# SysCV/sam-pt

Hardware: NVIDIA H100
Metric: frames/sec, SAM-PT hot path (PIPS track + SAM ViT encode + prompt/mask decode w/ 12 refinements) (higher is better)
Workload: dtype f16 hi.hi + two e4m3 correction passes (~fp32 products) qkv/MLP, f16 hi+lo x3 elsewhere ViT; f32 PIPS + decoder

## Files before the change

### sam-pt_b200/csrc/decoder.cu

```cuda
#include <cstdlib>

#include "common.cuh"
#include "kernels.cuh"
#include "tc_api.cuh"
#include "../../include/sampt_b200.h"

namespace sampt {

#define SKIP_RETURN(skip) \
  if ((skip) != nullptr && *(skip) != 0) return;

struct PromptArgs {
  const float* coords;
  const int* labels;
  int K;
  const float* box;
  int use_box;
  const float* gauss;
  const float* pt_emb[4];
  const float* not_a_point;
  const float* out_tokens;
  int n_out_tok;
  float img_size;
};
// ... 586 lines not shown
    const int w = threadIdx.x >> 5;
    if ((threadIdx.x & 31) == 0) { sred[0][w] = xmin; sred[1][w] = ymin; sred[2][w] = xmax; sred[3][w] = ymax; sred[4][w] = cnt; }
    __syncthreads();
    if (threadIdx.x == 0) {
      for (int k = 1; k < 8; ++k) {
        sred[0][0] = min(sred[0][0], sred[0][k]); sred[1][0] = min(sred[1][0], sred[1][k]);
        sred[2][0] = max(sred[2][0], sred[2][k]); sred[3][0] = max(sred[3][0], sred[3][k]);
        sred[4][0] += sred[4][k];
      }
      if (sred[4][0] > 0) {
        atomicMin(&bbox[0], sred[0][0]); atomicMin(&bbox[1], sred[1][0]);
        atomicMax(&bbox[2], sred[2][0]); atomicMax(&bbox[3], sred[3][0]);
        atomicAdd(&bbox[4], sred[4][0]);
      }
    }
  }
}
__global__ void refine_ctl_kernel(int* bbox, float* box_out, int* skip, int* n_done) {
  if (*skip == 0) {
    if (bbox[4] < 2) *skip = 1;
    else {
      box_out[0] = (float)bbox[0]; box_out[1] = (float)bbox[1]; box_out[2] = (float)bbox[2]; box_out[3] = (float)bbox[3];
      if (n_done) *n_done += 1;
    }
  }
  bbox[0] = 0x7fffffff; bbox[1] = 0x7fffffff; bbox[2] = -1; bbox[3] = -1; bbox[4] = 0;
}
__global__ void init_ctl_kernel(int* bbox, int* skip, int* n_done) {
  bbox[0] = 0x7fffffff; bbox[1] = 0x7fffffff; bbox[2] = -1; bbox[3] = -1; bbox[4] = 0;
  *skip = 0;
  if (n_done) *n_done = 0;
}

struct AttnW {
  const float *qw, *qb, *kw, *kb, *vw, *vb, *ow, *ob; int internal;
  const __half *qw16 = nullptr, *kw16 = nullptr, *vw16 = nullptr, *ow16 = nullptr;
};
struct LayerW {
  AttnW self_attn, t2i, i2t;
  const float *n1w, *n1b, *n2w, *n2b, *n3w, *n3b, *n4w, *n4b;
  const float *l1w, *l1b, *l2w, *l2b;
  const float *pek_t2i, *peq_i2t;
};
struct DecW {
  LayerW layer[2];
  AttnW final_attn; const float *nfw, *nfb, *pek_final;
  const float *up0_w , *up0_b4 ;
  const __half* up0_w16 = nullptr;
  bool tc = false;
  const float *up_lnw, *up_lnb, *up3_w, *up3_b;
  Mlp3Job hyper[4], iou;
  DenseW dense;
  PromptArgs prompt;
  int n_out_tok;
  int hq = 0;
  Mlp3Job hq_mlp;
  const float *mf0_w, *mf0_b, *mf_lnw, *mf_lnb, *mf3_w, *mf3_b;
  const float *enc0_w, *enc0_b4, *enc_lnw, *enc_lnb, *enc3_w, *enc3_b;
  const float *cv0_w, *cv0_b4, *cv_lnw, *cv_lnb, *cv3_w, *cv3_b;
  int vit_dim = 0;
};

static int load_attn(Ctx* c, const std::string& p, AttnW* a, int internal) {
  a->internal = internal;
  SAMPT_TRY(get_f32(c, p + "q_proj.weight", &a->qw)); SAMPT_TRY(get_f32(c, p + "q_proj.bias", &a->qb));
  SAMPT_TRY(get_f32(c, p + "k_proj.weight", &a->kw)); SAMPT_TRY(get_f32(c, p + "k_proj.bias", &a->kb));
  SAMPT_TRY(get_f32(c, p + "v_proj.weight", &a->vw)); SAMPT_TRY(get_f32(c, p + "v_proj.bias", &a->vb));
  SAMPT_TRY(get_f32(c, p + "out_proj.weight", &a->ow)); SAMPT_TRY(get_f32(c, p + "out_proj.bias", &a->ob));
  return 0;
}
static bool decoder_tc_enabled() {
  static const int on = [] { const char* e = std::getenv("SAMPT_DECODER_TC"); return (e != nullptr && e[0] == '0') ? 0 : 1; }();
  return on != 0;
}
static int load_w16(Ctx* c, const std::string& name, const __half** out) { return get_f16(c, name, out); }
static int load_mlp3(Ctx* c, const std::string& p, Mlp3Job* j, int n_out) {
  SAMPT_TRY(get_f32(c, p + "layers.0.weight", &j->w0)); SAMPT_TRY(get_f32(c, p + "layers.0.bias", &j->b0));
  SAMPT_TRY(get_f32(c, p + "layers.1.weight", &j->w1)); SAMPT_TRY(get_f32(c, p + "layers.1.bias", &j->b1));
  SAMPT_TRY(get_f32(c, p + "layers.2.weight", &j->w2)); SAMPT_TRY(get_f32(c, p + "layers.2.bias", &j->b2));
  j->n_out = n_out;
  return 0;
}
static int load_dec(Ctx* c, DecW* w) {
  const std::string md = "sam.mask_decoder.", tr = md + "transformer.", pe = "sam.prompt_encoder.";
  for (int i = 0; i < 2; ++i) {
    const std::string lp = tr + "layers." + std::to_string(i) + ".";
    LayerW& L = w->layer[i];
    SAMPT_TRY(load_attn(c, lp + "self_attn.", &L.self_attn, 256));
    SAMPT_TRY(load_attn(c, lp + "cross_attn_token_to_image.", &L.t2i, 128));
    SAMPT_TRY(load_attn(c, lp + "cross_attn_image_to_token.", &L.i2t, 128));
    SAMPT_TRY(get_f32(c, lp + "norm1.weight", &L.n1w)); SAMPT_TRY(get_f32(c, lp + "norm1.bias", &L.n1b));
    SAMPT_TRY(get_f32(c, lp + "norm2.weight", &L.n2w)); SAMPT_TRY(get_f32(c, lp + "norm2.bias", &L.n2b));
    SAMPT_TRY(get_f32(c, lp + "norm3.weight", &L.n3w)); SAMPT_TRY(get_f32(c, lp + "norm3.bias", &L.n3b));
    SAMPT_TRY(get_f32(c, lp + "norm4.weight", &L.n4w)); SAMPT_TRY(get_f32(c, lp + "norm4.bias", &L.n4b));
    SAMPT_TRY(get_f32(c, lp + "mlp.lin1.weight", &L.l1w)); SAMPT_TRY(get_f32(c, lp + "mlp.lin1.bias", &L.l1b));
    SAMPT_TRY(get_f32(c, lp + "mlp.lin2.weight", &L.l2w)); SAMPT_TRY(get_f32(c, lp + "mlp.lin2.bias", &L.l2b));
    SAMPT_TRY(get_f32(c, lp + "pek_t2i", &L.pek_t2i)); SAMPT_TRY(get_f32(c, lp + "peq_i2t", &L.peq_i2t));
  }
  SAMPT_TRY(load_attn(c, tr + "final_attn_token_to_image.", &w->final_attn, 128));
  w->tc = decoder_tc_enabled() && c->find(md + "output_upscaling.0.w16") != nullptr;
  if (w->tc) {
    for (int i = 0; i < 2; ++i) {
      const std::string lp = tr + "layers." + std::to_string(i) + ".";
      SAMPT_TRY(load_w16(c, lp + "cross_attn_token_to_image.k_proj.w16", &w->layer[i].t2i.kw16));
      SAMPT_TRY(load_w16(c, lp + "cross_attn_token_to_image.v_proj.w16", &w->layer[i].t2i.vw16));
      SAMPT_TRY(load_w16(c, lp + "cross_attn_image_to_token.q_proj.w16", &w->layer[i].i2t.qw16));
      SAMPT_TRY(load_w16(c, lp + "cross_attn_image_to_token.out_proj.w16", &w->layer[i].i2t.ow16));
    }
// ... 51 lines not shown
  int T;
};

#define LAUNCH_OK() do { c->launches++; SAMPT_LAUNCH_CHECK(); } while (0)

static int sg(Ctx* c, cudaStream_t st, const float* X, int ldx, const float* W, const float* b, const float* resid, int ldr,
              float* Y, int ldy, int M, int N, int K, int act, const int* skip) {
  return sgemm_nt_skip(c, st, X, ldx, W, K, b, resid, ldr, Y, ldy, M, N, K, act, skip);
}

__global__ void __launch_bounds__(256)
split_f32_kernel(const float* __restrict__ x, __half* __restrict__ out, long long n4 , int K, const int* skip) {
  SKIP_RETURN(skip);
  const long long i = (long long)blockIdx.x * 256 + threadIdx.x;
  if (i >= n4) return;
  const long long e = i * 4;
  const long long r = e / K;
  const int cidx = (int)(e % K);
  const float4 v = *reinterpret_cast<const float4*>(x + e);
  const __half2 h0 = __floats2half2_rn(v.x, v.y), h1 = __floats2half2_rn(v.z, v.w);
  const float2 f0 = __half22float2(h0), f1 = __half22float2(h1);
  const __half2 l0 = __floats2half2_rn(v.x - f0.x, v.y - f0.y), l1 = __floats2half2_rn(v.z - f1.x, v.w - f1.y);
  __half* o = out + r * 2 * K + cidx;
  *reinterpret_cast<uint2*>(o) = make_uint2(*reinterpret_cast<const uint32_t*>(&h0), *reinterpret_cast<const uint32_t*>(&h1));
  *reinterpret_cast<uint2*>(o + K) = make_uint2(*reinterpret_cast<const uint32_t*>(&l0), *reinterpret_cast<const uint32_t*>(&l1));
}
static int split_rows(Ctx* c, cudaStream_t st, const float* x, __half* out, int rows, int K, const int* skip) {
  const long long n4 = (long long)rows * K / 4;
  split_f32_kernel<<<cdiv(n4, 256), 256, 0, st>>>(x, out, n4, K, skip);
  c->launches++;
  SAMPT_LAUNCH_CHECK();
  return 0;
}
static int tcg(Ctx* c, cudaStream_t st, const __half* X16, const __half* W16, const float* b, const float* resid, float* Y, int ldy,
               int M, int N, int K, const int* skip) {
  GemmSeg seg{};
  seg.nseg = 3;
  seg.a_off[0] = 0; seg.b_off[0] = 0;
  seg.a_off[1] = K; seg.b_off[1] = 0;
  seg.a_off[2] = 0; seg.b_off[2] = K;
  GemmEpi ep{};
  ep.out32 = Y; ep.ldc = ldy; ep.bias = b; ep.resid = resid; ep.skip = skip;
  return gemm_tc(c, st, X16, 2 * K, W16, 2 * K, M, N, K, seg, ep);
}

static int launch_tok_self(Ctx* c, cudaStream_t st, int kind, const float* q, const float* k, const float* v, float* out, int T,
                           const int* skip) {
  if (kind == 1) {
    const size_t smem = ((size_t)2 * T * 33 + (size_t)8 * T + 8 * 32) * sizeof(float);
    SAMPT_CHECK(smem <= 200 * 1024, "too many prompt tokens (%d) for the token self-attention", T);
    SAMPT_TRY(ensure_func_smem(c, "attn_tok_self_kernel<32>", attn_tok_self_kernel<32>, 200 * 1024));
    attn_tok_self_kernel<32><<<dim3(cdiv(T, 32), 8), 256, smem, st>>>(q, k, v, out, T, 8, skip);
  } else {
    attn_q_small_kernel<32><<<dim3(T, 8), 256, 0, st>>>(q, k, v, out, T, 8, skip);
  }
  LAUNCH_OK();
  return 0;
}
static int launch_t2i(Ctx* c, cudaStream_t st, const float* q, const float* k, const float* v, float* part, float* out, int T, int Nk,
                      const int* skip) {
  constexpr int KPS = 256;
  const int nsplit = (Nk + KPS - 1) / KPS;
  attn_t2i_partial_kernel<16, KPS><<<dim3(nsplit, 8), 256, 0, st>>>(q, k, v, part, T, Nk, 8, skip);
  LAUNCH_OK();
  attn_t2i_combine_kernel<16><<<cdiv(T * 128, 128), 128, 0, st>>>(part, out, T, 8, nsplit, skip);
  LAUNCH_OK();
  return 0;
}
static int launch_i2t(Ctx* c, cudaStream_t st, const float* q, const float* k, const float* v, float* out, int N, int T, const int* skip) {
  attn_kv_small_kernel<16><<<cdiv((long long)cdiv(N, 32) * 8, 8), 256, 0, st>>>(q, k, v, out, N, T, 8, skip);
  LAUNCH_OK();
  return 0;
}

static int attn_tok_to_img(Ctx* c, cudaStream_t st, const AttnW& a, const float* q_in, const float* keys, const float* pek,
                           DecBufs& b, float* out , const float* resid, int GG, const int* skip) {
  const int T = b.T;
  SAMPT_TRY(sg(c, st, q_in, 256, a.qw, a.qb, nullptr, 0, b.tq, 128, T, 128, 256, 0, skip));
  if (a.kw16 != nullptr) {
    SAMPT_TRY(tcg(c, st, b.keys16, a.kw16, a.kb, pek, b.ik, 128, GG, 128, 256, skip));
    SAMPT_TRY(tcg(c, st, b.keys16, a.vw16, a.vb, nullptr, b.iv, 128, GG, 128, 256, skip));
  } else {
    SAMPT_TRY(sg(c, st, keys, 256, a.kw, a.kb, pek, 128, b.ik, 128, GG, 128, 256, 0, skip));
    SAMPT_TRY(sg(c, st, keys, 256, a.vw, a.vb, nullptr, 0, b.iv, 128, GG, 128, 256, 0, skip));
  }
  SAMPT_TRY(launch_t2i(c, st, b.tq, b.ik, b.iv, b.part, b.ta, T, GG, skip));
  SAMPT_TRY(sg(c, st, b.ta, 128, a.ow, a.ob, resid, 256, out, 256, T, 256, 128, 0, skip));
  return 0;
}

static int two_way_layer(Ctx* c, cudaStream_t st, const LayerW& L, int idx, DecBufs& b, int GG, const int* skip) {
  const int T = b.T;
  if (idx == 0) {
    SAMPT_TRY(sg(c, st, b.queries, 256, L.self_attn.qw, L.self_attn.qb, nullptr, 0, b.tq, 256, T, 256, 256, 0, skip));
    SAMPT_TRY(sg(c, st, b.queries, 256, L.self_attn.kw, L.self_attn.kb, nullptr, 0, b.tk, 256, T, 256, 256, 0, skip));
  } else {
    add_kernel<<<cdiv(T * 64, 256), 256, 0, st>>>(b.queries, b.tokens, b.qpe, (long long)T * 64, skip);
    LAUNCH_OK();
    SAMPT_TRY(sg(c, st, b.qpe, 256, L.self_attn.qw, L.self_attn.qb, nullptr, 0, b.tq, 256, T, 256, 256, 0, skip));
    SAMPT_TRY(sg(c, st, b.qpe, 256, L.self_attn.kw, L.self_attn.kb, nullptr, 0, b.tk, 256, T, 256, 256, 0, skip));
  }
  SAMPT_TRY(sg(c, st, b.queries, 256, L.self_attn.vw, L.self_attn.vb, nullptr, 0, b.tv, 256, T, 256, 256, 0, skip));
  SAMPT_TRY(launch_tok_self(c, st, T > 16 ? 1 : 0, b.tq, b.tk, b.tv, b.ta, T, skip));
  SAMPT_TRY(sg(c, st, b.ta, 256, L.self_attn.ow, L.self_attn.ob, idx == 0 ? nullptr : b.queries, 256, b.tmp, 256, T, 256, 256, 0, skip));
  ln256_kernel<<<cdiv(T, 8), 256, 0, st>>>(b.tmp, nullptr, L.n1w, L.n1b, b.queries, T, 1e-5f, skip);
  LAUNCH_OK();
  add_kernel<<<cdiv(T * 64, 256), 256, 0, st>>>(b.queries, b.tokens, b.qpe, (long long)T * 64, skip);
  LAUNCH_OK();
  SAMPT_TRY(attn_tok_to_img(c, st, L.t2i, b.qpe, b.keys, L.pek_t2i, b, b.tmp, b.queries, GG, skip));
  ln256_kernel<<<cdiv(T, 8), 256, 0, st>>>(b.tmp, nullptr, L.n2w, L.n2b, b.queries, T, 1e-5f, skip);
  LAUNCH_OK();
  SAMPT_TRY(sg(c, st, b.queries, 256, L.l1w, L.l1b, nullptr, 0, b.mlp_h, 2048, T, 2048, 256, 2, skip));
  SAMPT_TRY(sg(c, st, b.mlp_h, 2048, L.l2w, L.l2b, b.queries, 256, b.tmp, 256, T, 256, 2048, 0, skip));
  ln256_kernel<<<cdiv(T, 8), 256, 0, st>>>(b.tmp, nullptr, L.n3w, L.n3b, b.queries, T, 1e-5f, skip);
  LAUNCH_OK();
  add_kernel<<<cdiv(T * 64, 256), 256, 0, st>>>(b.queries, b.tokens, b.qpe, (long long)T * 64, skip);
  LAUNCH_OK();
  if (L.i2t.qw16 != nullptr) SAMPT_TRY(tcg(c, st, b.keys16, L.i2t.qw16, L.i2t.qb, L.peq_i2t, b.iq, 128, GG, 128, 256, skip));
  else SAMPT_TRY(sg(c, st, b.keys, 256, L.i2t.qw, L.i2t.qb, L.peq_i2t, 128, b.iq, 128, GG, 128, 256, 0, skip));
  SAMPT_TRY(sg(c, st, b.qpe, 256, L.i2t.kw, L.i2t.kb, nullptr, 0, b.tk, 128, T, 128, 256, 0, skip));
  SAMPT_TRY(sg(c, st, b.queries, 256, L.i2t.vw, L.i2t.vb, nullptr, 0, b.tv, 128, T, 128, 256, 0, skip));
  SAMPT_TRY(launch_i2t(c, st, b.iq, b.tk, b.tv, b.ia, GG, T, skip));
  if (L.i2t.ow16 != nullptr) {
    SAMPT_TRY(split_rows(c, st, b.ia, b.ia16, GG, 128, skip));
    SAMPT_TRY(tcg(c, st, b.ia16, L.i2t.ow16, L.i2t.ob, b.keys, b.src, 256, GG, 256, 128, skip));
  } else {
    SAMPT_TRY(sg(c, st, b.ia, 128, L.i2t.ow, L.i2t.ob, b.keys, 256, b.src, 256, GG, 256, 128, 0, skip));
  }
  ln256_kernel<<<cdiv(GG, 8), 256, 0, st>>>(b.src, nullptr, L.n4w, L.n4b, b.keys, GG, 1e-5f, skip);
  LAUNCH_OK();
  if (L.i2t.ow16 != nullptr) SAMPT_TRY(split_rows(c, st, b.keys, b.keys16, GG, 256, skip));
  return 0;
}

struct DecodeCall {
  const float* feat_tok;
  const float* coords; const int* labels; int K;
  const float* box; int use_box;
  const float* mask_in;
  int n_masks, tok0;
  int in_h, in_w, H, W;
  float* logits;
  float* iou;
  float* low_res;
  int* bbox;
  const int* skip;
  const float* hq_feat;
};

static int encode_prompt(Ctx* c, cudaStream_t st, const DecW& w, const DecodeCall& d, int G, float* tokens, float* src) {
  const int T = w.n_out_tok + d.K + (d.use_box ? 2 : 1);
  PromptArgs pa = w.prompt;
  pa.coords = d.coords; pa.labels = d.labels; pa.K = d.K; pa.box = d.box; pa.use_box = d.use_box; pa.img_size = (float)(G * 16);
  prompt_tokens_kernel<<<T, 256, 0, st>>>(pa, tokens, d.skip);
  LAUNCH_OK();
  dense_src_kernel<<<cdiv(G * G, 8), 256, 0, st>>>(d.feat_tok, d.mask_in, w.dense, src, G, d.skip);
  LAUNCH_OK();
  return 0;
}
static int launch_upscale(Ctx* c, cudaStream_t st, const DecW& w, const float* u1, const float* hyper, int n_masks, float* low_res,
                          int G, float* u_out, const int* skip) {
  upscale_mask_kernel<<<cdiv(16 * G * G, 256), 256, 0, st>>>(u1, w.up_lnw, w.up_lnb, w.up3_w, w.up3_b, hyper, n_masks, low_res, G,
                                                             u_out, skip);
  LAUNCH_OK();
// ... 422 lines not shown
```

### sam-pt_b200/csrc/gemm_tc.cu

```cuda
#include "common.cuh"
#include "tc_common.cuh"
#include "kernels.cuh"
#include "tc_api.cuh"
#include "../../include/sampt_b200.h"

namespace sampt {

using namespace tc;

constexpr int G_BM = 128, G_BN = 128, G_BK = 64, G_STAGES = 3;
constexpr int G_A_BYTES = G_BM * G_BK * 2;
constexpr int G_B_BYTES = G_BN * G_BK * 2;
constexpr int G_STAGE_BYTES = G_A_BYTES + G_B_BYTES;
constexpr int G_SMEM_BYTES = G_STAGES * G_STAGE_BYTES + 1024  + 256 ;
constexpr int G_THREADS = 288;

__global__ void __launch_bounds__(G_THREADS, 2)
gemm_tc_kernel(const __grid_constant__ CUtensorMap tmA, const __grid_constant__ CUtensorMap tmB, int M, int N, int K,
               GemmSeg seg, GemmEpi ep) {
  if (ep.skip != nullptr && *ep.skip != 0) return;
  extern __shared__ uint8_t smem_raw[];
  uint8_t* smem = reinterpret_cast<uint8_t*>((reinterpret_cast<uintptr_t>(smem_raw) + 1023) & ~uintptr_t(1023));
  uint64_t* full_bar = reinterpret_cast<uint64_t*>(smem + G_STAGES * G_STAGE_BYTES);
  uint64_t* empty_bar = full_bar + G_STAGES;

  const int warp = threadIdx.x >> 5, lane = threadIdx.x & 31;
  const int n_tiles = (N + G_BN - 1) / G_BN;
  const int m_blk = blockIdx.x / n_tiles, n_blk = blockIdx.x % n_tiles;
  int seg_kb[3];
#pragma unroll
  for (int i = 0; i < 3; ++i) seg_kb[i] = i < seg.nseg ? (seg.f8[i] ? K / (2 * G_BK) : K / G_BK) : 0;

  if (threadIdx.x == 0) {
    for (int i = 0; i < G_STAGES; ++i) { mbar_init(&full_bar[i], 1); mbar_init(&empty_bar[i], 256); }
    fence_barrier_init();
  }
  __syncthreads();

  if (warp == 8) {
    if (lane == 0) {
      tma_prefetch_desc(&tmA);
      tma_prefetch_desc(&tmB);
      uint32_t it = 0;
      for (int sg = 0; sg < seg.nseg; ++sg) {
        for (int kb = 0; kb < seg_kb[sg]; ++kb, ++it) {
          const int s = it % G_STAGES;
          const uint32_t ph = (it / G_STAGES) & 1;
          mbar_wait(&empty_bar[s], ph ^ 1);
          const int kk = kb * G_BK;
          uint8_t* sa = smem + s * G_STAGE_BYTES;
          mbar_expect_tx(&full_bar[s], G_STAGE_BYTES);
          tma_load_2d(sa, &tmA, &full_bar[s], seg.a_off[sg] + kk, m_blk * G_BM);
          tma_load_2d(sa + G_A_BYTES, &tmB, &full_bar[s], seg.b_off[sg] + kk, n_blk * G_BN);
        }
      }
    }
    return;
  }

  const int g = warp >> 2, w = warp & 3;
  float acc[64];
#pragma unroll
  for (int i = 0; i < 64; ++i) acc[i] = 0.f;
  uint32_t it = 0;
  int prev_s = -1;
  for (int sg = 0; sg < seg.nseg; ++sg) {
    const bool f8 = seg.f8[sg] != 0;
    for (int kb = 0; kb < seg_kb[sg]; ++kb, ++it) {
      const int s = it % G_STAGES;
      mbar_wait(&full_bar[s], (it / G_STAGES) & 1);
      const uint32_t sa = smem_u32(smem + s * G_STAGE_BYTES);
      const uint64_t adesc = make_smem_desc_sw128(sa + g * 64 * 128);
      const uint64_t bdesc = make_smem_desc_sw128(sa + G_A_BYTES);
      wgmma_fence();
      if (f8) {
#pragma unroll
        for (int k = 0; k < 4; ++k) wgmma_m64n128k32_e4m3(acc, adesc + (uint64_t)(2 * k), bdesc + (uint64_t)(2 * k));
      } else if (ep.is_bf16) {
#pragma unroll
        for (int k = 0; k < 4; ++k) wgmma_m64n128k16_bf16(acc, adesc + (uint64_t)(2 * k), bdesc + (uint64_t)(2 * k));
      } else {
#pragma unroll
        for (int k = 0; k < 4; ++k) wgmma_m64n128k16_f16(acc, adesc + (uint64_t)(2 * k), bdesc + (uint64_t)(2 * k));
      }
      wgmma_commit();
      wgmma_wait<1>();
      if (prev_s >= 0) mbar_arrive(&empty_bar[prev_s]);
      prev_s = s;
    }
  }
  wgmma_wait<0>();
  wgmma_fence_regs(acc);

  const float acc_scale = ep.acc_scale ? __ldg(ep.acc_scale) : 1.0f;
  const int c2 = 2 * (lane & 3);
#pragma unroll
  for (int h = 0; h < 2; ++h) {
    const int m = m_blk * G_BM + g * 64 + w * 16 + (lane >> 2) + 8 * h;
    if (m >= M) continue;
    long long drow = m;
    if (ep.rowmap) drow = ep.rowmap[m];
    if (drow < 0) continue;
#pragma unroll
    for (int i = 0; i < G_BN / 8; ++i) {
      const int n = n_blk * G_BN + 8 * i + c2;
      if (n >= N) continue;
      float v0 = acc[4 * i + 2 * h], v1 = acc[4 * i + 2 * h + 1];
      v0 *= acc_scale; v1 *= acc_scale;
      if (ep.bias) { v0 += __ldg(ep.bias + n); v1 += __ldg(ep.bias + n + 1); }
      if (ep.act == 1) { v0 = gelu_erf(v0); v1 = gelu_erf(v1); }
      else if (ep.act == 3) { v0 = gelu_tanh(v0); v1 = gelu_tanh(v1); }
      if (ep.out32) {
        float* o = ep.out32 + (size_t)drow * ep.ldc + n;
        if (ep.resid) {
          const long long rrow = ep.resid_mod > 0 ? (drow % ep.resid_mod) : drow;
          const float2 t = *reinterpret_cast<const float2*>(ep.resid + (size_t)rrow * ep.ldc + n);
          v0 += t.x; v1 += t.y;
        }
        *reinterpret_cast<float2*>(o) = make_float2(v0, v1);
      } else if (ep.is_bf16) {
        *reinterpret_cast<__nv_bfloat162*>(ep.out16 + (size_t)drow * ep.ldc + n) = __floats2bfloat162_rn(v0, v1);
      } else {
        __half* o = ep.out16 + (size_t)drow * ep.ldc + n;
        const __half2 hv = __floats2half2_rn(v0, v1);
        *reinterpret_cast<__half2*>(o) = hv;
        const float2 hf = __half22float2(hv);
        if (ep.split_off > 0 && ep.out_f8) {
          uint8_t* ob = reinterpret_cast<uint8_t*>(ep.out16 + (size_t)drow * ep.ldc + ep.split_off) + n;
          uint16_t l8, h8;
          asm("cvt.rn.satfinite.e4m3x2.f32 %0, %1, %2;" : "=h"(l8) : "f"((v1 - hf.y) * F8_LO_SCALE), "f"((v0 - hf.x) * F8_LO_SCALE));
          asm("cvt.rn.satfinite.e4m3x2.f32 %0, %1, %2;" : "=h"(h8) : "f"(v1 * F8_HI_SCALE), "f"(v0 * F8_HI_SCALE));
          *reinterpret_cast<uint16_t*>(ob) = l8;
          *reinterpret_cast<uint16_t*>(ob + ep.split_off) = h8;
        } else if (ep.split_off > 0) {
          *reinterpret_cast<__half2*>(o + ep.split_off) = __floats2half2_rn(v0 - hf.x, v1 - hf.y);
        }
      }
    }
  }
}

bool gemm_f8c_applicable(int M, int N, int K) { return M >= 256 && N % 256 == 0 && K % (2 * G_BK) == 0; }

int gemm_tc(Ctx* c, cudaStream_t st, const void* A, int lda, const void* B, int ldb, int M, int N, int K, const GemmSeg& seg,
            const GemmEpi& ep) {
  SAMPT_CHECK(K % G_BK == 0 && K > 0, "gemm_tc: K (%d) must be a positive multiple of %d", K, G_BK);
  SAMPT_CHECK(N % 32 == 0, "gemm_tc: N (%d) must be a multiple of 32", N);
  SAMPT_CHECK(seg.nseg >= 1 && seg.nseg <= 3, "gemm_tc: nseg out of range");
  SAMPT_CHECK((ep.out16 != nullptr) != (ep.out32 != nullptr), "gemm_tc: exactly one of out16/out32 must be set");
  SAMPT_CHECK(ep.ldc % 8 == 0, "gemm_tc: ldc must be a multiple of 8");
  SAMPT_CHECK(ep.act == 0 || ep.act == 1 || ep.act == 3, "gemm_tc: act %d is not 0 (none), 1 (GELU erf) or 3 (GELU tanh)", ep.act);
  const bool f8 = (seg.f8[0] | seg.f8[1] | seg.f8[2]) != 0;
  SAMPT_CHECK(!f8 || K % (2 * G_BK) == 0, "gemm_tc: e4m3 segments need K %% 128 == 0 (K = %d)", K);
  SAMPT_CHECK(!f8 || !ep.is_bf16, "gemm_tc: e4m3 segments go with fp16 operands");
  CUtensorMap tmA, tmB;
  SAMPT_TRY(make_tmap_2d_f16(&tmA, A, (uint64_t)lda, (uint64_t)M, (uint64_t)lda * 2, G_BK, G_BM));
  SAMPT_TRY(make_tmap_2d_f16(&tmB, B, (uint64_t)ldb, (uint64_t)N, (uint64_t)ldb * 2, G_BK, G_BN));
  const int m_tiles = (M + G_BM - 1) / G_BM, n_tiles = (N + G_BN - 1) / G_BN;
  const int grid = m_tiles * n_tiles;
  GemmSeg ord{};
  ord.nseg = seg.nseg;
  int j = 0;
  for (int pass = 1; pass >= 0; --pass)
    for (int i = 0; i < seg.nseg; ++i)
      if ((seg.f8[i] != 0) == (pass == 1)) { ord.a_off[j] = seg.a_off[i]; ord.b_off[j] = seg.b_off[i]; ord.f8[j] = seg.f8[i]; ++j; }
  SAMPT_TRY(ensure_func_smem(c, "gemm_tc_kernel", gemm_tc_kernel, G_SMEM_BYTES));
  gemm_tc_kernel<<<grid, G_THREADS, G_SMEM_BYTES, st>>>(tmA, tmB, M, N, K, ord, ep);
  c->launches++;
  SAMPT_LAUNCH_CHECK();
  return 0;
}

}

using namespace sampt;

extern "C" int sampt_gemm_f16(sampt_ctx* ctx, const void* A, int lda, const void* B, int ldb, int M, int N, int K, int precision,
                              int is_bf16, const float* bias, int act, void* out16, float* out32, const float* resid, int ldc,
                              int split_off, void* stream) {
  Ctx* c = reinterpret_cast<Ctx*>(ctx);
  GemmSeg seg{};
  seg.nseg = precision;
  SAMPT_CHECK(precision >= 1 && precision <= 3, "precision must be 1, 2 or 3");
  if (precision == 2) {
    seg.a_off[0] = 0; seg.b_off[0] = 0;
    seg.a_off[1] = 0; seg.b_off[1] = K;
  } else {
    seg.a_off[0] = 0; seg.b_off[0] = 0;
    seg.a_off[1] = K; seg.b_off[1] = 0;
    seg.a_off[2] = 0; seg.b_off[2] = K;
// ... 63 lines not shown
```

### sam-pt_b200/csrc/tc_common.cuh

```cuda
#pragma once
#include <cuda.h>
#include <cuda_runtime.h>
#include <cstdint>

namespace sampt {
namespace tc {

__device__ __forceinline__ uint32_t smem_u32(const void* p) { return (uint32_t)__cvta_generic_to_shared(p); }

__device__ __forceinline__ void mbar_init(uint64_t* bar, uint32_t count) {
  asm volatile("mbarrier.init.shared::cta.b64 [%0], %1;" ::"r"(smem_u32(bar)), "r"(count));
}
__device__ __forceinline__ void fence_barrier_init() { asm volatile("fence.mbarrier_init.release.cluster;" ::: "memory"); }
__device__ __forceinline__ void fence_proxy_async() { asm volatile("fence.proxy.async.shared::cta;" ::: "memory"); }
__device__ __forceinline__ void mbar_expect_tx(uint64_t* bar, uint32_t bytes) {
  asm volatile("mbarrier.arrive.expect_tx.shared::cta.b64 _, [%0], %1;" ::"r"(smem_u32(bar)), "r"(bytes) : "memory");
}
__device__ __forceinline__ void mbar_arrive(uint64_t* bar) {
  asm volatile("mbarrier.arrive.shared::cta.b64 _, [%0];" ::"r"(smem_u32(bar)) : "memory");
}
__device__ __forceinline__ uint32_t mbar_try_wait(uint64_t* bar, uint32_t parity) {
  uint32_t ok;
  asm volatile(
      "{\n"
      ".reg .pred p;\n"
      "mbarrier.try_wait.parity.shared::cta.b64 p, [%1], %2;\n"
      "selp.b32 %0, 1, 0, p;\n"
      "}\n"
      : "=r"(ok)
      : "r"(smem_u32(bar)), "r"(parity)
      : "memory");
  return ok;
}
__device__ __forceinline__ void mbar_wait(uint64_t* bar, uint32_t parity) {
  while (!mbar_try_wait(bar, parity)) {
  }
}

__device__ __forceinline__ void tma_prefetch_desc(const CUtensorMap* m) {
  asm volatile("prefetch.tensormap [%0];" ::"l"(reinterpret_cast<uint64_t>(m)) : "memory");
}
__device__ __forceinline__ void tma_load_2d(void* smem_dst, const CUtensorMap* m, uint64_t* bar, int c0, int c1) {
  asm volatile(
      "cp.async.bulk.tensor.2d.shared::cluster.global.mbarrier::complete_tx::bytes [%0], [%1, {%3, %4}], [%2];" ::"r"(
          smem_u32(smem_dst)),
      "l"(reinterpret_cast<uint64_t>(m)), "r"(smem_u32(bar)), "r"(c0), "r"(c1)
      : "memory");
}
__device__ __forceinline__ void tma_load_3d(void* smem_dst, const CUtensorMap* m, uint64_t* bar, int c0, int c1, int c2) {
  asm volatile(
      "cp.async.bulk.tensor.3d.shared::cluster.global.mbarrier::complete_tx::bytes [%0], [%1, {%3, %4, %5}], [%2];" ::"r"(
          smem_u32(smem_dst)),
      "l"(reinterpret_cast<uint64_t>(m)), "r"(smem_u32(bar)), "r"(c0), "r"(c1), "r"(c2)
      : "memory");
}

__device__ __forceinline__ void wgmma_fence() { asm volatile("wgmma.fence.sync.aligned;" ::: "memory"); }
__device__ __forceinline__ void wgmma_commit() { asm volatile("wgmma.commit_group.sync.aligned;" ::: "memory"); }
template <int N>
__device__ __forceinline__ void wgmma_wait() { asm volatile("wgmma.wait_group.sync.aligned %0;" ::"n"(N) : "memory"); }
template <int R>
__device__ __forceinline__ void wgmma_fence_regs(float (&d)[R]) {
#pragma unroll
  for (int i = 0; i < R; ++i) asm volatile("" : "+f"(d[i])::"memory");
}

__device__ __forceinline__ void wgmma_m64n128k16_f16(float (&d)[64], uint64_t da, uint64_t db) {
  asm volatile(
      "{\n.reg .pred p;\nsetp.ne.b32 p, %66, 0;\n"
      "wgmma.mma_async.sync.aligned.m64n128k16.f32.f16.f16 {%0, %1, %2, %3, %4, %5, %6, %7, %8, %9, %10, %11, %12, %13, %14, %15, %16, %17, %18, %19, %20, %21, %22, %23, %24, %25, %26, %27, %28, %29, %30, %31, %32, %33, %34, %35, %36, %37, %38, %39, %40, %41, %42, %43, %44, %45, %46, %47, %48, %49, %50, %51, %52, %53, %54, %55, %56, %57, %58, %59, %60, %61, %62, %63}, %64, %65, p, 1, 1, 0, 0;\n}\n"
      : "+f"(d[0]), "+f"(d[1]), "+f"(d[2]), "+f"(d[3]), "+f"(d[4]), "+f"(d[5]), "+f"(d[6]), "+f"(d[7]), "+f"(d[8]), "+f"(d[9]), "+f"(d[10]), "+f"(d[11]), "+f"(d[12]), "+f"(d[13]), "+f"(d[14]), "+f"(d[15]), "+f"(d[16]), "+f"(d[17]), "+f"(d[18]), "+f"(d[19]), "+f"(d[20]), "+f"(d[21]), "+f"(d[22]), "+f"(d[23]), "+f"(d[24]), "+f"(d[25]), "+f"(d[26]), "+f"(d[27]), "+f"(d[28]), "+f"(d[29]), "+f"(d[30]), "+f"(d[31]), "+f"(d[32]), "+f"(d[33]), "+f"(d[34]), "+f"(d[35]), "+f"(d[36]), "+f"(d[37]), "+f"(d[38]), "+f"(d[39]), "+f"(d[40]), "+f"(d[41]), "+f"(d[42]), "+f"(d[43]), "+f"(d[44]), "+f"(d[45]), "+f"(d[46]), "+f"(d[47]), "+f"(d[48]), "+f"(d[49]), "+f"(d[50]), "+f"(d[51]), "+f"(d[52]), "+f"(d[53]), "+f"(d[54]), "+f"(d[55]), "+f"(d[56]), "+f"(d[57]), "+f"(d[58]), "+f"(d[59]), "+f"(d[60]), "+f"(d[61]), "+f"(d[62]), "+f"(d[63])
      : "l"(da), "l"(db), "r"(1));
}

__device__ __forceinline__ void wgmma_m64n128k16_bf16(float (&d)[64], uint64_t da, uint64_t db) {
  asm volatile(
      "{\n.reg .pred p;\nsetp.ne.b32 p, %66, 0;\n"
      "wgmma.mma_async.sync.aligned.m64n128k16.f32.bf16.bf16 {%0, %1, %2, %3, %4, %5, %6, %7, %8, %9, %10, %11, %12, %13, %14, %15, %16, %17, %18, %19, %20, %21, %22, %23, %24, %25, %26, %27, %28, %29, %30, %31, %32, %33, %34, %35, %36, %37, %38, %39, %40, %41, %42, %43, %44, %45, %46, %47, %48, %49, %50, %51, %52, %53, %54, %55, %56, %57, %58, %59, %60, %61, %62, %63}, %64, %65, p, 1, 1, 0, 0;\n}\n"
      : "+f"(d[0]), "+f"(d[1]), "+f"(d[2]), "+f"(d[3]), "+f"(d[4]), "+f"(d[5]), "+f"(d[6]), "+f"(d[7]), "+f"(d[8]), "+f"(d[9]), "+f"(d[10]), "+f"(d[11]), "+f"(d[12]), "+f"(d[13]), "+f"(d[14]), "+f"(d[15]), "+f"(d[16]), "+f"(d[17]), "+f"(d[18]), "+f"(d[19]), "+f"(d[20]), "+f"(d[21]), "+f"(d[22]), "+f"(d[23]), "+f"(d[24]), "+f"(d[25]), "+f"(d[26]), "+f"(d[27]), "+f"(d[28]), "+f"(d[29]), "+f"(d[30]), "+f"(d[31]), "+f"(d[32]), "+f"(d[33]), "+f"(d[34]), "+f"(d[35]), "+f"(d[36]), "+f"(d[37]), "+f"(d[38]), "+f"(d[39]), "+f"(d[40]), "+f"(d[41]), "+f"(d[42]), "+f"(d[43]), "+f"(d[44]), "+f"(d[45]), "+f"(d[46]), "+f"(d[47]), "+f"(d[48]), "+f"(d[49]), "+f"(d[50]), "+f"(d[51]), "+f"(d[52]), "+f"(d[53]), "+f"(d[54]), "+f"(d[55]), "+f"(d[56]), "+f"(d[57]), "+f"(d[58]), "+f"(d[59]), "+f"(d[60]), "+f"(d[61]), "+f"(d[62]), "+f"(d[63])
      : "l"(da), "l"(db), "r"(1));
}

__device__ __forceinline__ void wgmma_m64n128k32_e4m3(float (&d)[64], uint64_t da, uint64_t db) {
  asm volatile(
      "{\n.reg .pred p;\nsetp.ne.b32 p, %66, 0;\n"
      "wgmma.mma_async.sync.aligned.m64n128k32.f32.e4m3.e4m3 {%0, %1, %2, %3, %4, %5, %6, %7, %8, %9, %10, %11, %12, %13, %14, %15, %16, %17, %18, %19, %20, %21, %22, %23, %24, %25, %26, %27, %28, %29, %30, %31, %32, %33, %34, %35, %36, %37, %38, %39, %40, %41, %42, %43, %44, %45, %46, %47, %48, %49, %50, %51, %52, %53, %54, %55, %56, %57, %58, %59, %60, %61, %62, %63}, %64, %65, p, 1, 1;\n}\n"
      : "+f"(d[0]), "+f"(d[1]), "+f"(d[2]), "+f"(d[3]), "+f"(d[4]), "+f"(d[5]), "+f"(d[6]), "+f"(d[7]), "+f"(d[8]), "+f"(d[9]), "+f"(d[10]), "+f"(d[11]), "+f"(d[12]), "+f"(d[13]), "+f"(d[14]), "+f"(d[15]), "+f"(d[16]), "+f"(d[17]), "+f"(d[18]), "+f"(d[19]), "+f"(d[20]), "+f"(d[21]), "+f"(d[22]), "+f"(d[23]), "+f"(d[24]), "+f"(d[25]), "+f"(d[26]), "+f"(d[27]), "+f"(d[28]), "+f"(d[29]), "+f"(d[30]), "+f"(d[31]), "+f"(d[32]), "+f"(d[33]), "+f"(d[34]), "+f"(d[35]), "+f"(d[36]), "+f"(d[37]), "+f"(d[38]), "+f"(d[39]), "+f"(d[40]), "+f"(d[41]), "+f"(d[42]), "+f"(d[43]), "+f"(d[44]), "+f"(d[45]), "+f"(d[46]), "+f"(d[47]), "+f"(d[48]), "+f"(d[49]), "+f"(d[50]), "+f"(d[51]), "+f"(d[52]), "+f"(d[53]), "+f"(d[54]), "+f"(d[55]), "+f"(d[56]), "+f"(d[57]), "+f"(d[58]), "+f"(d[59]), "+f"(d[60]), "+f"(d[61]), "+f"(d[62]), "+f"(d[63])
// ... 74 lines not shown
```

### sam-pt_b200/segment_anything/modeling/sam.py

```python
import os
from typing import List

import torch
from torch import nn

from sampt_b200 import native


class Sam(nn.Module):
    mask_threshold: float = 0.0
    image_format: str = "RGB"

    def __init__(self, image_encoder, prompt_encoder, mask_decoder, pixel_mean: List[float] = (123.675, 116.28, 103.53),
                 pixel_std: List[float] = (58.395, 57.12, 57.375)) -> None:
        super().__init__()
        self.image_encoder = image_encoder
        self.prompt_encoder = prompt_encoder
        self.mask_decoder = mask_decoder
        self.register_buffer("pixel_mean", torch.tensor(list(pixel_mean), dtype=torch.float32).view(-1, 1, 1), False)
        self.register_buffer("pixel_std", torch.tensor(list(pixel_std), dtype=torch.float32).view(-1, 1, 1), False)
        self._dec_registered = None
        self.use_cuda_graphs = os.environ.get("SAMPT_DECODE_GRAPHS", "1") != "0"

    @property
    def device(self):
        return self.pixel_mean.device

    def has_decoder_slab(self) -> bool:
        return bool(self.use_cuda_graphs)

    def native_context(self) -> native.Context:
        ctx = self.image_encoder.native_context()
        key = (id(ctx), tuple(p._version for p in self.prompt_encoder.parameters()),
               tuple(p._version for p in self.mask_decoder.parameters()), self.device)
        if self._dec_registered != key or not ctx.owns("sam.decoder", self):
            self._register_decoder(ctx)
            if self.use_cuda_graphs:
                ctx.set_decoder_workspace()
            else:
                ctx.clear_decoder_workspace()
            self._dec_registered = key
            ctx.claim("sam.decoder", self)
        return ctx

    @torch.no_grad()
    def _register_decoder(self, ctx: native.Context) -> None:
        pe, md = self.prompt_encoder, self.mask_decoder
        torch.cuda.synchronize(ctx.device)
        ctx.unset_prefix("sam.prompt_encoder.")
        ctx.unset_prefix("sam.mask_decoder.")
        for k, v in pe.state_dict().items():
            ctx.set_tensor("sam.prompt_encoder." + k, v.float().reshape(-1) if v.dim() == 2 and v.shape[0] == 1 else v.float())
        sd = md.state_dict()
        for k, v in sd.items():
            ctx.set_tensor("sam.mask_decoder." + k, v.float())
        toks = [sd["iou_token.weight"], sd["mask_tokens.weight"]]
        if "hf_token.weight" in sd:
            toks.append(sd["hf_token.weight"])
        ctx.set_tensor("sam.mask_decoder.output_tokens", torch.cat(toks, dim=0).float())
        w0 = sd["output_upscaling.0.weight"].float()
        ctx.set_tensor("sam.mask_decoder.output_upscaling.0.weight_gemm", w0.permute(2, 3, 1, 0).reshape(-1, w0.shape[0]))
        ctx.set_tensor("sam.mask_decoder.output_upscaling.0.bias4", sd["output_upscaling.0.bias"].float().repeat(4))

        def w16(wm):
            wm = wm.float()
            hi = wm.half()
            return torch.cat([hi, (wm - hi.float()).half()], dim=1).contiguous()

        ctx.set_tensor("sam.mask_decoder.output_upscaling.0.w16", w16(w0.permute(2, 3, 1, 0).reshape(-1, w0.shape[0])))
        for name in [f"transformer.layers.{i}.cross_attn_token_to_image.{p}_proj" for i in range(2) for p in ("k", "v")] + \
                    [f"transformer.layers.{i}.cross_attn_image_to_token.{p}_proj" for i in range(2) for p in ("q", "out")] + \
                    [f"transformer.final_attn_token_to_image.{p}_proj" for p in ("k", "v")]:
            ctx.set_tensor(f"sam.mask_decoder.{name}.w16", w16(sd[name + ".weight"]))
        dense_pe = pe.get_dense_pe()[0].flatten(1).t().contiguous()
        ctx.set_tensor("sam.dense_pe_tok", dense_pe)
        t = "sam.mask_decoder.transformer."
        for i in range(2):
            wk = sd[f"transformer.layers.{i}.cross_attn_token_to_image.k_proj.weight"].float()
            wq = sd[f"transformer.layers.{i}.cross_attn_image_to_token.q_proj.weight"].float()
            ctx.set_tensor(f"{t}layers.{i}.pek_t2i", dense_pe @ wk.t())
            ctx.set_tensor(f"{t}layers.{i}.peq_i2t", dense_pe @ wq.t())
        wk = sd["transformer.final_attn_token_to_image.k_proj.weight"].float()
        ctx.set_tensor(f"{t}pek_final", dense_pe @ wk.t())

    def forward(self, batched_input, multimask_output):
        raise NotImplementedError("use SamPredictor (set_image / predict_torch); the batched dict interface of upstream "
                                  "Sam.forward is not on the SAM-PT hot path")
```

Before: 23.77.

## Stage GEMM epilogue through shared memory and disable decoder tensor-core path by default

Rewrites the tensor-core GEMM epilogue to stage accumulator tiles through swizzled shared memory in 32-column chunks. Each chunk is then written with 16-byte coalesced stores, with residual adds done on float4, synchronised by named barriers. The k-loop is refactored into a templated helper. Decoder tensor-core GEMM weights gain a per-tensor scale loaded from the encoder's split helper. The decoder tensor-core path now defaults to off unless SAMPT_DECODER_TC=1, so the decoder falls back to the f32 SIMT GEMMs. The ViT GEMMs benefit from the coalesced epilogue at the cost of extra shared-memory traffic and barriers.

Measured after the change: 25.38 (median of 6 runs). +6.8%, better.

```diff
diff --git a/sam-pt_b200/csrc/decoder.cu b/sam-pt_b200/csrc/decoder.cu
--- a/sam-pt_b200/csrc/decoder.cu
+++ b/sam-pt_b200/csrc/decoder.cu
@@ -642,9 +642,10 @@
   if (n_done) *n_done = 0;
 }
 
+struct W16 { const __half* w = nullptr; const float* s = nullptr; };
 struct AttnW {
   const float *qw, *qb, *kw, *kb, *vw, *vb, *ow, *ob; int internal;
-  const __half *qw16 = nullptr, *kw16 = nullptr, *vw16 = nullptr, *ow16 = nullptr;
+  W16 qw16, kw16, vw16, ow16;
 };
 struct LayerW {
   AttnW self_attn, t2i, i2t;
@@ -656,7 +657,7 @@
   LayerW layer[2];
   AttnW final_attn; const float *nfw, *nfb, *pek_final;
   const float *up0_w , *up0_b4 ;
-  const __half* up0_w16 = nullptr;
+  W16 up0_w16;
   bool tc = false;
   const float *up_lnw, *up_lnb, *up3_w, *up3_b;
   Mlp3Job hyper[4], iou;
@@ -680,10 +681,13 @@
   return 0;
 }
 static bool decoder_tc_enabled() {
-  static const int on = [] { const char* e = std::getenv("SAMPT_DECODER_TC"); return (e != nullptr && e[0] == '0') ? 0 : 1; }();
+  static const int on = [] { const char* e = std::getenv("SAMPT_DECODER_TC"); return (e != nullptr && e[0] == '1') ? 1 : 0; }();
   return on != 0;
 }
-static int load_w16(Ctx* c, const std::string& name, const __half** out) { return get_f16(c, name, out); }
+static int load_w16(Ctx* c, const std::string& name, W16* out) {
+  SAMPT_TRY(get_f16(c, name, &out->w));
+  return get_f32(c, name + "s", &out->s);
+}
 static int load_mlp3(Ctx* c, const std::string& p, Mlp3Job* j, int n_out) {
   SAMPT_TRY(get_f32(c, p + "layers.0.weight", &j->w0)); SAMPT_TRY(get_f32(c, p + "layers.0.bias", &j->b0));
   SAMPT_TRY(get_f32(c, p + "layers.1.weight", &j->w1)); SAMPT_TRY(get_f32(c, p + "layers.1.bias", &j->b1));
@@ -801,7 +805,7 @@
   SAMPT_LAUNCH_CHECK();
   return 0;
 }
-static int tcg(Ctx* c, cudaStream_t st, const __half* X16, const __half* W16, const float* b, const float* resid, float* Y, int ldy,
+static int tcg(Ctx* c, cudaStream_t st, const __half* X16, const W16& W, const float* b, const float* resid, float* Y, int ldy,
                int M, int N, int K, const int* skip) {
   GemmSeg seg{};
   seg.nseg = 3;
@@ -809,8 +813,8 @@
   seg.a_off[1] = K; seg.b_off[1] = 0;
   seg.a_off[2] = 0; seg.b_off[2] = K;
   GemmEpi ep{};
-  ep.out32 = Y; ep.ldc = ldy; ep.bias = b; ep.resid = resid; ep.skip = skip;
-  return gemm_tc(c, st, X16, 2 * K, W16, 2 * K, M, N, K, seg, ep);
+  ep.out32 = Y; ep.ldc = ldy; ep.bias = b; ep.resid = resid; ep.skip = skip; ep.acc_scale = W.s;
+  return gemm_tc(c, st, X16, 2 * K, W.w, 2 * K, M, N, K, seg, ep);
 }
 
 static int launch_tok_self(Ctx* c, cudaStream_t st, int kind, const float* q, const float* k, const float* v, float* out, int T,
@@ -846,7 +850,7 @@
                            DecBufs& b, float* out , const float* resid, int GG, const int* skip) {
   const int T = b.T;
   SAMPT_TRY(sg(c, st, q_in, 256, a.qw, a.qb, nullptr, 0, b.tq, 128, T, 128, 256, 0, skip));
-  if (a.kw16 != nullptr) {
+  if (a.kw16.w != nullptr) {
     SAMPT_TRY(tcg(c, st, b.keys16, a.kw16, a.kb, pek, b.ik, 128, GG, 128, 256, skip));
     SAMPT_TRY(tcg(c, st, b.keys16, a.vw16, a.vb, nullptr, b.iv, 128, GG, 128, 256, skip));
   } else {
@@ -885,12 +889,12 @@
   LAUNCH_OK();
   add_kernel<<<cdiv(T * 64, 256), 256, 0, st>>>(b.queries, b.tokens, b.qpe, (long long)T * 64, skip);
   LAUNCH_OK();
-  if (L.i2t.qw16 != nullptr) SAMPT_TRY(tcg(c, st, b.keys16, L.i2t.qw16, L.i2t.qb, L.peq_i2t, b.iq, 128, GG, 128, 256, skip));
+  if (L.i2t.qw16.w != nullptr) SAMPT_TRY(tcg(c, st, b.keys16, L.i2t.qw16, L.i2t.qb, L.peq_i2t, b.iq, 128, GG, 128, 256, skip));
   else SAMPT_TRY(sg(c, st, b.keys, 256, L.i2t.qw, L.i2t.qb, L.peq_i2t, 128, b.iq, 128, GG, 128, 256, 0, skip));
   SAMPT_TRY(sg(c, st, b.qpe, 256, L.i2t.kw, L.i2t.kb, nullptr, 0, b.tk, 128, T, 128, 256, 0, skip));
   SAMPT_TRY(sg(c, st, b.queries, 256, L.i2t.vw, L.i2t.vb, nullptr, 0, b.tv, 128, T, 128, 256, 0, skip));
   SAMPT_TRY(launch_i2t(c, st, b.iq, b.tk, b.tv, b.ia, GG, T, skip));
-  if (L.i2t.ow16 != nullptr) {
+  if (L.i2t.ow16.w != nullptr) {
     SAMPT_TRY(split_rows(c, st, b.ia, b.ia16, GG, 128, skip));
     SAMPT_TRY(tcg(c, st, b.ia16, L.i2t.ow16, L.i2t.ob, b.keys, b.src, 256, GG, 256, 128, skip));
   } else {
@@ -898,7 +902,7 @@
   }
   ln256_kernel<<<cdiv(GG, 8), 256, 0, st>>>(b.src, nullptr, L.n4w, L.n4b, b.keys, GG, 1e-5f, skip);
   LAUNCH_OK();
-  if (L.i2t.ow16 != nullptr) SAMPT_TRY(split_rows(c, st, b.keys, b.keys16, GG, 256, skip));
+  if (L.i2t.ow16.w != nullptr) SAMPT_TRY(split_rows(c, st, b.keys, b.keys16, GG, 256, skip));
   return 0;
 }
 
diff --git a/sam-pt_b200/csrc/gemm_tc.cu b/sam-pt_b200/csrc/gemm_tc.cu
--- a/sam-pt_b200/csrc/gemm_tc.cu
+++ b/sam-pt_b200/csrc/gemm_tc.cu
@@ -12,8 +12,120 @@
 constexpr int G_A_BYTES = G_BM * G_BK * 2;
 constexpr int G_B_BYTES = G_BN * G_BK * 2;
 constexpr int G_STAGE_BYTES = G_A_BYTES + G_B_BYTES;
+constexpr int G_EPI_COLS = 32;
 constexpr int G_SMEM_BYTES = G_STAGES * G_STAGE_BYTES + 1024  + 256 ;
 constexpr int G_THREADS = 288;
+constexpr int G_BAR_RING = 1;
+constexpr int G_BAR_EPI = 2;
+
+__device__ __forceinline__ uint8_t* stg_at(uint8_t* stg, int r, int u) { return stg + r * 128 + ((u ^ (r & 7)) << 4); }
+
+template <int NH>
+__device__ __forceinline__ void gemm_epilogue(float (&acc)[NH][64], uint8_t* stg, int h0, int m0, int n0, int M, int N,
+                                              const GemmEpi& ep, float acc_scale, int w, int lane, int bar) {
+  const int c2 = 2 * (lane & 3);
+#pragma unroll
+  for (int ch = 0; ch < G_BN / G_EPI_COLS; ++ch) {
+    const int nc = n0 + ch * G_EPI_COLS;
+    if (nc >= N) break;
+#pragma unroll
+    for (int hh = 0; hh < NH; ++hh) {
+#pragma unroll
+      for (int h = 0; h < 2; ++h) {
+        const int r = (h0 + hh) * 64 + w * 16 + (lane >> 2) + 8 * h;
+#pragma unroll
+        for (int q = 0; q < 4; ++q) {
+          const int i = ch * 4 + q;
+          const int n = nc + 8 * q + c2;
+          float v0 = acc[hh][4 * i + 2 * h], v1 = acc[hh][4 * i + 2 * h + 1];
+          v0 = __fmul_rn(v0, acc_scale); v1 = __fmul_rn(v1, acc_scale);
+          if (ep.bias) { v0 = __fadd_rn(v0, __ldg(ep.bias + n)); v1 = __fadd_rn(v1, __ldg(ep.bias + n + 1)); }
+          if (ep.act == 1) { v0 = gelu_erf(v0); v1 = gelu_erf(v1); }
+          else if (ep.act == 3) { v0 = gelu_tanh(v0); v1 = gelu_tanh(v1); }
+          const int j = 8 * q + c2;
+          if (ep.out32) {
+            *reinterpret_cast<float2*>(stg_at(stg, r, j >> 2) + 4 * (j & 3)) = make_float2(v0, v1);
+          } else if (ep.is_bf16) {
+            *reinterpret_cast<__nv_bfloat162*>(stg_at(stg, r, q) + 2 * c2) = __floats2bfloat162_rn(v0, v1);
+          } else {
+            const __half2 hv = __floats2half2_rn(v0, v1);
+            *reinterpret_cast<__half2*>(stg_at(stg, r, q) + 2 * c2) = hv;
+            const float2 hf = __half22float2(hv);
+            if (ep.split_off > 0 && ep.out_f8) {
+              uint16_t l8, h8;
+              asm("cvt.rn.satfinite.e4m3x2.f32 %0, %1, %2;" : "=h"(l8) : "f"((v1 - hf.y) * F8_LO_SCALE), "f"((v0 - hf.x) * F8_LO_SCALE));
+              asm("cvt.rn.satfinite.e4m3x2.f32 %0, %1, %2;" : "=h"(h8) : "f"(v1 * F8_HI_SCALE), "f"(v0 * F8_HI_SCALE));
+              *reinterpret_cast<uint16_t*>(stg_at(stg, r, 4 + (q >> 1)) + 8 * (q & 1) + c2) = l8;
+              *reinterpret_cast<uint16_t*>(stg_at(stg, r, 6 + (q >> 1)) + 8 * (q & 1) + c2) = h8;
+            } else if (ep.split_off > 0) {
+              *reinterpret_cast<__half2*>(stg_at(stg, r, 4 + q) + 2 * c2) = __floats2half2_rn(v0 - hf.x, v1 - hf.y);
+            }
+          }
+        }
+      }
+    }
+    named_bar_sync(bar, 128);
+#pragma unroll
+    for (int k = 0; k < 4 * NH; ++k) {
+      const int r = h0 * 64 + w * 16 * NH + 4 * k + (lane >> 3), u = lane & 7;
+      const int m = m0 + r;
+      if (m >= M) continue;
+      long long drow = m;
+      if (ep.rowmap) drow = ep.rowmap[m];
+      if (drow < 0) continue;
+      const uint4 val = *reinterpret_cast<const uint4*>(stg_at(stg, r, u));
+      if (ep.out32) {
+        const int n = nc + 4 * u;
+        float4 v = *reinterpret_cast<const float4*>(&val);
+        if (ep.resid) {
+          const long long rrow = ep.resid_mod > 0 ? (drow % ep.resid_mod) : drow;
+          const float4 t = *reinterpret_cast<const float4*>(ep.resid + (size_t)rrow * ep.ldc + n);
+          v.x = __fadd_rn(v.x, t.x); v.y = __fadd_rn(v.y, t.y); v.z = __fadd_rn(v.z, t.z); v.w = __fadd_rn(v.w, t.w);
+        }
+        *reinterpret_cast<float4*>(ep.out32 + (size_t)drow * ep.ldc + n) = v;
+      } else {
+        __half* orow = ep.out16 + (size_t)drow * ep.ldc;
+        if (u < 4) {
+          *reinterpret_cast<uint4*>(orow + nc + 8 * u) = val;
+        } else if (ep.split_off > 0 && !ep.is_bf16) {
+          if (ep.out_f8) {
+            uint8_t* ob = reinterpret_cast<uint8_t*>(orow + ep.split_off) + nc + (u < 6 ? 16 * (u - 4) : ep.split_off + 16 * (u - 6));
+            *reinterpret_cast<uint4*>(ob) = val;
+          } else {
+            *reinterpret_cast<uint4*>(orow + ep.split_off + nc + 8 * (u - 4)) = val;
+          }
+        }
+      }
+    }
+    named_bar_sync(bar, 128);
+  }
+}
+
+template <int NH, int KIND>
+__device__ __forceinline__ void gemm_kloop(float (&acc)[NH][64], uint8_t* smem, uint64_t* full_bar, uint64_t* empty_bar, int nkb,
+                                           int h0, uint32_t& it, int& prev_s) {
+  for (int kb = 0; kb < nkb; ++kb, ++it) {
+    const int s = it % G_STAGES;
+    mbar_wait(&full_bar[s], (it / G_STAGES) & 1);
+    const uint32_t sa = smem_u32(smem + s * G_STAGE_BYTES);
+    const uint64_t bdesc = make_smem_desc_sw128(sa + G_A_BYTES);
+    wgmma_fence();
+#pragma unroll
+    for (int hh = 0; hh < NH; ++hh) {
+      const uint64_t adesc = make_smem_desc_sw128(sa + (h0 + hh) * 64 * 128);
+#pragma unroll
+      for (int k = 0; k < 4; ++k) {
+        if (KIND == 0) wgmma_m64n128k32_e4m3(acc[hh], adesc + (uint64_t)(2 * k), bdesc + (uint64_t)(2 * k));
+        else if (KIND == 1) wgmma_m64n128k16_bf16(acc[hh], adesc + (uint64_t)(2 * k), bdesc + (uint64_t)(2 * k));
+        else wgmma_m64n128k16_f16(acc[hh], adesc + (uint64_t)(2 * k), bdesc + (uint64_t)(2 * k));
+      }
+    }
+    wgmma_commit();
+    wgmma_wait<1>();
+    if (prev_s >= 0) mbar_arrive(&empty_bar[prev_s]);
+    prev_s = s;
+  }
+}
 
 __global__ void __launch_bounds__(G_THREADS, 2)
 gemm_tc_kernel(const __grid_constant__ CUtensorMap tmA, const __grid_constant__ CUtensorMap tmB, int M, int N, int K,
@@ -59,85 +171,21 @@
   }
 
   const int g = warp >> 2, w = warp & 3;
-  float acc[64];
-#pragma unroll
-  for (int i = 0; i < 64; ++i) acc[i] = 0.f;
+  float acc[1][64];
+#pragma unroll
+  for (int i = 0; i < 64; ++i) acc[0][i] = 0.f;
   uint32_t it = 0;
   int prev_s = -1;
   for (int sg = 0; sg < seg.nseg; ++sg) {
-    const bool f8 = seg.f8[sg] != 0;
-    for (int kb = 0; kb < seg_kb[sg]; ++kb, ++it) {
-      const int s = it % G_STAGES;
-      mbar_wait(&full_bar[s], (it / G_STAGES) & 1);
-      const uint32_t sa = smem_u32(smem + s * G_STAGE_BYTES);
-      const uint64_t adesc = make_smem_desc_sw128(sa + g * 64 * 128);
-      const uint64_t bdesc = make_smem_desc_sw128(sa + G_A_BYTES);
-      wgmma_fence();
-      if (f8) {
-#pragma unroll
-        for (int k = 0; k < 4; ++k) wgmma_m64n128k32_e4m3(acc, adesc + (uint64_t)(2 * k), bdesc + (uint64_t)(2 * k));
-      } else if (ep.is_bf16) {
-#pragma unroll
-        for (int k = 0; k < 4; ++k) wgmma_m64n128k16_bf16(acc, adesc + (uint64_t)(2 * k), bdesc + (uint64_t)(2 * k));
-      } else {
-#pragma unroll
-        for (int k = 0; k < 4; ++k) wgmma_m64n128k16_f16(acc, adesc + (uint64_t)(2 * k), bdesc + (uint64_t)(2 * k));
-      }
-      wgmma_commit();
-      wgmma_wait<1>();
-      if (prev_s >= 0) mbar_arrive(&empty_bar[prev_s]);
-      prev_s = s;
-    }
+    if (seg.f8[sg]) gemm_kloop<1, 0>(acc, smem, full_bar, empty_bar, seg_kb[sg], g, it, prev_s);
+    else if (ep.is_bf16) gemm_kloop<1, 1>(acc, smem, full_bar, empty_bar, seg_kb[sg], g, it, prev_s);
+    else gemm_kloop<1, 2>(acc, smem, full_bar, empty_bar, seg_kb[sg], g, it, prev_s);
   }
   wgmma_wait<0>();
-  wgmma_fence_regs(acc);
-
+  wgmma_fence_regs(acc[0]);
+  named_bar_sync(G_BAR_RING, 256);
   const float acc_scale = ep.acc_scale ? __ldg(ep.acc_scale) : 1.0f;
-  const int c2 = 2 * (lane & 3);
-#pragma unroll
-  for (int h = 0; h < 2; ++h) {
-    const int m = m_blk * G_BM + g * 64 + w * 16 + (lane >> 2) + 8 * h;
-    if (m >= M) continue;
-    long long drow = m;
-    if (ep.rowmap) drow = ep.rowmap[m];
-    if (drow < 0) continue;
-#pragma unroll
-    for (int i = 0; i < G_BN / 8; ++i) {
-      const int n = n_blk * G_BN + 8 * i + c2;
-      if (n >= N) continue;
-      float v0 = acc[4 * i + 2 * h], v1 = acc[4 * i + 2 * h + 1];
-      v0 *= acc_scale; v1 *= acc_scale;
-      if (ep.bias) { v0 += __ldg(ep.bias + n); v1 += __ldg(ep.bias + n + 1); }
-      if (ep.act == 1) { v0 = gelu_erf(v0); v1 = gelu_erf(v1); }
-      else if (ep.act == 3) { v0 = gelu_tanh(v0); v1 = gelu_tanh(v1); }
-      if (ep.out32) {
-        float* o = ep.out32 + (size_t)drow * ep.ldc + n;
-        if (ep.resid) {
-          const long long rrow = ep.resid_mod > 0 ? (drow % ep.resid_mod) : drow;
-          const float2 t = *reinterpret_cast<const float2*>(ep.resid + (size_t)rrow * ep.ldc + n);
-          v0 += t.x; v1 += t.y;
-        }
-        *reinterpret_cast<float2*>(o) = make_float2(v0, v1);
-      } else if (ep.is_bf16) {
-        *reinterpret_cast<__nv_bfloat162*>(ep.out16 + (size_t)drow * ep.ldc + n) = __floats2bfloat162_rn(v0, v1);
-      } else {
-        __half* o = ep.out16 + (size_t)drow * ep.ldc + n;
-        const __half2 hv = __floats2half2_rn(v0, v1);
-        *reinterpret_cast<__half2*>(o) = hv;
-        const float2 hf = __half22float2(hv);
-        if (ep.split_off > 0 && ep.out_f8) {
-          uint8_t* ob = reinterpret_cast<uint8_t*>(ep.out16 + (size_t)drow * ep.ldc + ep.split_off) + n;
-          uint16_t l8, h8;
-          asm("cvt.rn.satfinite.e4m3x2.f32 %0, %1, %2;" : "=h"(l8) : "f"((v1 - hf.y) * F8_LO_SCALE), "f"((v0 - hf.x) * F8_LO_SCALE));
-          asm("cvt.rn.satfinite.e4m3x2.f32 %0, %1, %2;" : "=h"(h8) : "f"(v1 * F8_HI_SCALE), "f"(v0 * F8_HI_SCALE));
-          *reinterpret_cast<uint16_t*>(ob) = l8;
-          *reinterpret_cast<uint16_t*>(ob + ep.split_off) = h8;
-        } else if (ep.split_off > 0) {
-          *reinterpret_cast<__half2*>(o + ep.split_off) = __floats2half2_rn(v0 - hf.x, v1 - hf.y);
-        }
-      }
-    }
-  }
+  gemm_epilogue<1>(acc, smem, g, m_blk * G_BM, n_blk * G_BN, M, N, ep, acc_scale, w, lane, G_BAR_EPI + g);
 }
 
 bool gemm_f8c_applicable(int M, int N, int K) { return M >= 256 && N % 256 == 0 && K % (2 * G_BK) == 0; }
@@ -156,6 +204,10 @@
   CUtensorMap tmA, tmB;
   SAMPT_TRY(make_tmap_2d_f16(&tmA, A, (uint64_t)lda, (uint64_t)M, (uint64_t)lda * 2, G_BK, G_BM));
   SAMPT_TRY(make_tmap_2d_f16(&tmB, B, (uint64_t)ldb, (uint64_t)N, (uint64_t)ldb * 2, G_BK, G_BN));
+  auto al16 = [](const void* p) { return (reinterpret_cast<uintptr_t>(p) & 15) == 0; };
+  SAMPT_CHECK(al16(ep.out16) && al16(ep.out32) && al16(ep.resid), "gemm_tc: output and residual must be 16-byte aligned");
+  SAMPT_CHECK(ep.split_off % (ep.out_f8 ? 16 : 8) == 0, "gemm_tc: split_off (%d) must be a multiple of %d", ep.split_off,
+              ep.out_f8 ? 16 : 8);
   const int m_tiles = (M + G_BM - 1) / G_BM, n_tiles = (N + G_BN - 1) / G_BN;
   const int grid = m_tiles * n_tiles;
   GemmSeg ord{};
diff --git a/sam-pt_b200/csrc/tc_common.cuh b/sam-pt_b200/csrc/tc_common.cuh
--- a/sam-pt_b200/csrc/tc_common.cuh
+++ b/sam-pt_b200/csrc/tc_common.cuh
@@ -53,6 +53,10 @@
           smem_u32(smem_dst)),
       "l"(reinterpret_cast<uint64_t>(m)), "r"(smem_u32(bar)), "r"(c0), "r"(c1), "r"(c2)
       : "memory");
+}
+
+__device__ __forceinline__ void named_bar_sync(int id, int count) {
+  asm volatile("bar.sync %0, %1;" ::"r"(id), "r"(count) : "memory");
 }
 
 __device__ __forceinline__ void wgmma_fence() { asm volatile("wgmma.fence.sync.aligned;" ::: "memory"); }
diff --git a/sam-pt_b200/segment_anything/modeling/sam.py b/sam-pt_b200/segment_anything/modeling/sam.py
--- a/sam-pt_b200/segment_anything/modeling/sam.py
+++ b/sam-pt_b200/segment_anything/modeling/sam.py
@@ -5,6 +5,8 @@
 from torch import nn
 
 from sampt_b200 import native
+
+from .image_encoder import ImageEncoderViT
 
 
 class Sam(nn.Module):
@@ -62,16 +64,16 @@
         ctx.set_tensor("sam.mask_decoder.output_upscaling.0.weight_gemm", w0.permute(2, 3, 1, 0).reshape(-1, w0.shape[0]))
         ctx.set_tensor("sam.mask_decoder.output_upscaling.0.bias4", sd["output_upscaling.0.bias"].float().repeat(4))
 
-        def w16(wm):
-            wm = wm.float()
-            hi = wm.half()
-            return torch.cat([hi, (wm - hi.float()).half()], dim=1).contiguous()
+        def w16(name, wm):
+            w, scale = ImageEncoderViT._w16(wm, True)
+            ctx.set_tensor(name + ".w16", w)
+            ctx.set_tensor(name + ".w16s", scale)
 
-        ctx.set_tensor("sam.mask_decoder.output_upscaling.0.w16", w16(w0.permute(2, 3, 1, 0).reshape(-1, w0.shape[0])))
+        w16("sam.mask_decoder.output_upscaling.0", w0.permute(2, 3, 1, 0).reshape(-1, w0.shape[0]))
         for name in [f"transformer.layers.{i}.cross_attn_token_to_image.{p}_proj" for i in range(2) for p in ("k", "v")] + \
                     [f"transformer.layers.{i}.cross_attn_image_to_token.{p}_proj" for i in range(2) for p in ("q", "out")] + \
                     [f"transformer.final_attn_token_to_image.{p}_proj" for p in ("k", "v")]:
-            ctx.set_tensor(f"sam.mask_decoder.{name}.w16", w16(sd[name + ".weight"]))
+            w16(f"sam.mask_decoder.{name}", sd[name + ".weight"])
         dense_pe = pe.get_dense_pe()[0].flatten(1).t().contiguous()
         ctx.set_tensor("sam.dense_pe_tok", dense_pe)
         t = "sam.mask_decoder.transformer."
```
